# rampasek/GraphGPS

Hardware: NVIDIA H100
Metric: graphs/sec GPSLayer fwd+bwd (higher is better)
Workload: dtype f32

## Files before the change

### graphgps_b200/csrc/attention.cu

```cuda
#include "kernels.cuh"

namespace gps {

namespace {

constexpr int kWarpsPerBlock = 4;

__device__ __forceinline__ int find_graph(const int* __restrict__ gptr, int B, int node) {
  int lo = 0, hi = B;
  while (hi - lo > 1) {
    int mid = (lo + hi) >> 1;
    if (gptr[mid] <= node) lo = mid; else hi = mid;
  }
  return lo;
}

template <int LPR>
__device__ __forceinline__ float group_sum(float v) {
#pragma unroll
  for (int o = LPR / 2; o > 0; o >>= 1) v += __shfl_xor_sync(0xffffffffu, v, o);
  return v;
}

__device__ __forceinline__ int warp_max_i(int v) {
#pragma unroll
  for (int o = 16; o > 0; o >>= 1) v = max(v, __shfl_xor_sync(0xffffffffu, v, o));
  return v;
}

struct DropQuad {
  Philox4 r;
  uint32_t thr;
  float keep_scale;
};
__device__ __forceinline__ void drop_quad_refresh(DropQuad& q, float p, uint64_t seed, uint64_t offset, int head, int i, int jl) {
  q.r = philox4x32(seed, offset + (uint64_t)(GPS_SITE_ATTN_P + head), ((uint64_t)i << 20) | (uint64_t)(jl >> 2));
}
__device__ __forceinline__ float drop_quad_scale(const DropQuad& q, int jl) {
  const int k = jl & 3;
  const uint32_t bits = k == 0 ? q.r.v[0] : k == 1 ? q.r.v[1] : k == 2 ? q.r.v[2] : q.r.v[3];
  return bits >= q.thr ? q.keep_scale : 0.f;
}
__device__ __forceinline__ void drop_quad_init(DropQuad& q, float p) {
  q.thr = (uint32_t)fminf(p * 4294967296.f, 4294967295.f);
  q.keep_scale = 1.f / (1.f - p);
}

template <int VW> struct VecT;
template <> struct VecT<4> { using T = float4; };
template <> struct VecT<1> { using T = float; };

template <int VW> __device__ __forceinline__ typename VecT<VW>::T vld(const float* p);
template <> __device__ __forceinline__ float4 vld<4>(const float* p) { return ld4(p); }
template <> __device__ __forceinline__ float vld<1>(const float* p) { return *p; }
template <int VW> __device__ __forceinline__ typename VecT<VW>::T vzero();
template <> __device__ __forceinline__ float4 vzero<4>() { return f4zero(); }
template <> __device__ __forceinline__ float vzero<1>() { return 0.f; }
__device__ __forceinline__ void vst(float* p, float4 v) { st4(p, v); }
__device__ __forceinline__ void vst(float* p, float v) { *p = v; }
__device__ __forceinline__ float4 vscale(float4 a, float s) { return f4scale(a, s); }
__device__ __forceinline__ float vscale(float a, float s) { return a * s; }
__device__ __forceinline__ float vdot(float4 a, float4 b) { return a.x * b.x + a.y * b.y + a.z * b.z + a.w * b.w; }
__device__ __forceinline__ float vdot(float a, float b) { return a * b; }
__device__ __forceinline__ void vplanes_store(const Planes& p, int64_t r, int64_t c, float4 v) { planes_store4(p, r, c, v); }
__device__ __forceinline__ void vplanes_store(const Planes& p, int64_t r, int64_t c, float v) {
  const __nv_bfloat16 h = __float2bfloat16_rn(v);
  p.hi[r * p.ld + c] = h;
  if (p.lo) p.lo[r * p.ld + c] = __float2bfloat16_rn(v - __bfloat162float(h));
}

template <int CH, int LPR, int VW>
__device__ __forceinline__ void load_slice(typename VecT<VW>::T* dst, const float* row, int sub, int nch, bool ok) {
#pragma unroll
  for (int c = 0; c < CH; ++c) {
    int ch = sub + c * LPR;
    dst[c] = (ok && ch < nch) ? vld<VW>(row + ch * VW) : vzero<VW>();
  }
}
template <int CH, int LPR, int VW>
__device__ __forceinline__ void store_slice(const typename VecT<VW>::T* src, float* row, int sub, int nch) {
#pragma unroll
  for (int c = 0; c < CH; ++c) {
    int ch = sub + c * LPR;
    if (ch < nch) vst(row + ch * VW, src[c]);
  }
}
template <int CH, int LPR, int VW>
__device__ __forceinline__ void store_slice_planes(const typename VecT<VW>::T* src, const Planes& p, int64_t r, int64_t col0,
                                                   int sub, int nch) {
  if (!p.hi) return;
#pragma unroll
  for (int c = 0; c < CH; ++c) {
    int ch = sub + c * LPR;
    if (ch < nch) vplanes_store(p, r, col0 + ch * VW, src[c]);
  }
}
template <int CH, typename V>
__device__ __forceinline__ float dot_slice(const V* a, const V* b) {
  float s = 0.f;
#pragma unroll
  for (int c = 0; c < CH; ++c) s += vdot(a[c], b[c]);
  return s;
}

struct AttnArgs {
  const int* gptr; int B; int N; int H; int hd;
  const float* Q; const float* K; const float* V; int64_t ld;
  float* O; const float* Oc; const float* dO; int64_t ldo;
  float* lse; const float* lsec; float* delta; const float* deltac;
  float* dQ; float* dK; float* dV; int64_t ldg;
  float scale; float p_drop; uint64_t seed, offset;
  const unsigned long long* offset_dev;
  Planes Op, dQp, dKp, dVp;
  int smem_rows;
  const float* bias; int64_t nmax; float* gbias;
};
__device__ __forceinline__ uint64_t eff_offset(const AttnArgs& a) {
  return a.offset + ((a.p_drop > 0.f && a.offset_dev) ? *a.offset_dev : 0ull);
}

struct StagedRows {
  const float* x; int64_t ldx;
  const float* y; int64_t ldy;
};
template <int RPB, int VW>
__device__ __forceinline__ StagedRows stage_rows(const AttnArgs& a, const float* X, int64_t ldX, const float* Y, int64_t ldY,
                                                 int h, float* sm) {
  const int64_t hoff = (int64_t)h * a.hd;
  StagedRows r{X + hoff, ldX, Y + hoff, ldY};
  const int r0 = blockIdx.x * RPB;
  if (a.smem_rows <= 0 || r0 >= a.N) return r;
  const int last = min(r0 + RPB, a.N) - 1;
  const int kmin = a.gptr[find_graph(a.gptr, a.B, r0)];
  const int R = a.gptr[find_graph(a.gptr, a.B, last) + 1] - kmin;
  if (R > a.smem_rows) return r;
  const int pitch = a.hd + 4, nch = VW == 4 ? a.hd >> 2 : a.hd;
  float* sx = sm;
  float* sy = sm + (int64_t)a.smem_rows * pitch;
  for (int idx = threadIdx.x; idx < R * nch; idx += blockDim.x) {
    const int row = idx / nch, c = idx - row * nch;
    vst(sx + row * pitch + c * VW, vld<VW>(X + (int64_t)(kmin + row) * ldX + hoff + c * VW));
    vst(sy + row * pitch + c * VW, vld<VW>(Y + (int64_t)(kmin + row) * ldY + hoff + c * VW));
  }
  __syncthreads();
  r.x = sx - (int64_t)kmin * pitch; r.ldx = pitch;
  r.y = sy - (int64_t)kmin * pitch; r.ldy = pitch;
  return r;
}

template <int CH, int LPR, bool BIAS, int VW>
__global__ void __launch_bounds__(kWarpsPerBlock * 32) k_attn_fwd(AttnArgs a) {
  extern __shared__ float attn_sm[];
  using V = typename VecT<VW>::T;
  constexpr int RPW = 32 / LPR;
  const int warp = threadIdx.x >> 5, lane = threadIdx.x & 31;
  const int sub = lane % LPR, rloc = lane / LPR;
  const int h = blockIdx.y;
  const int i = (blockIdx.x * kWarpsPerBlock + warp) * RPW + rloc;
  const bool row_ok = i < a.N;
  const int nch = a.hd / VW;
  const uint64_t offs = eff_offset(a);
  int gs = 0, n = 0;
  const float* brow = nullptr;
  if (row_ok) {
    int g = find_graph(a.gptr, a.B, i);
    gs = a.gptr[g];
    n = a.gptr[g + 1] - gs;
    if constexpr (BIAS) brow = a.bias + (((int64_t)g * a.H + h) * a.nmax + (i - gs)) * a.nmax;
  }
  const int nloop = warp_max_i(n);
  const int64_t hoff = (int64_t)h * a.hd;
  V q[CH], o[CH];
  load_slice<CH, LPR, VW>(q, a.Q + (int64_t)(row_ok ? i : 0) * a.ld + hoff, sub, nch, row_ok);
#pragma unroll
  for (int c = 0; c < CH; ++c) {
    q[c] = vscale(q[c], a.scale);
    o[c] = vzero<VW>();
  }
  float m = -INFINITY, l = 0.f;
  const bool use_drop = a.p_drop > 0.f;
  DropQuad dq;
  drop_quad_init(dq, a.p_drop);
  const StagedRows kv = stage_rows<RPW * kWarpsPerBlock, VW>(a, a.K, a.ld, a.V, a.ld, h, attn_sm);
  V kc[CH], vc[CH];
  load_slice<CH, LPR, VW>(kc, kv.x + (int64_t)gs * kv.ldx, sub, nch, n > 0);
  load_slice<CH, LPR, VW>(vc, kv.y + (int64_t)gs * kv.ldy, sub, nch, n > 0);
  float bc = 0.f;
  if constexpr (BIAS) bc = n > 0 ? brow[0] : 0.f;
  for (int jl = 0; jl < nloop; ++jl) {
    if (use_drop && (jl & 3) == 0) drop_quad_refresh(dq, a.p_drop, a.seed, offs, h, i, jl);
    const bool valid = jl < n;
    const bool nvalid = jl + 1 < n;
    const int jn = gs + (nvalid ? jl + 1 : 0);
    V kn[CH], vn[CH];
    load_slice<CH, LPR, VW>(kn, kv.x + (int64_t)jn * kv.ldx, sub, nch, nvalid);
    load_slice<CH, LPR, VW>(vn, kv.y + (int64_t)jn * kv.ldy, sub, nch, nvalid);
    float bn = 0.f;
    if constexpr (BIAS) bn = nvalid ? brow[jl + 1] : 0.f;
    float s = group_sum<LPR>(dot_slice<CH>(q, kc));
    if constexpr (BIAS) s += bc;
    s = valid ? s : -INFINITY;
    const float m_new = fmaxf(m, s);
    const float corr = (m_new == -INFINITY) ? 1.f : __expf(m - m_new);
    const float p = valid ? __expf(s - m_new) : 0.f;
    l = l * corr + p;
    const float pd = use_drop ? p * drop_quad_scale(dq, jl) : p;
#pragma unroll
    for (int c = 0; c < CH; ++c) {
      if constexpr (VW == 4) {
        o[c].x = o[c].x * corr + pd * vc[c].x;
        o[c].y = o[c].y * corr + pd * vc[c].y;
        o[c].z = o[c].z * corr + pd * vc[c].z;
        o[c].w = o[c].w * corr + pd * vc[c].w;
      } else {
        o[c] = o[c] * corr + pd * vc[c];
      }
      kc[c] = kn[c];
      vc[c] = vn[c];
    }
    if constexpr (BIAS) bc = bn;
    m = m_new;
  }
  if (row_ok) {
    const float inv = 1.f / l;
#pragma unroll
    for (int c = 0; c < CH; ++c) o[c] = vscale(o[c], inv);
    store_slice<CH, LPR, VW>(o, a.O + (int64_t)i * a.ldo + hoff, sub, nch);
    store_slice_planes<CH, LPR, VW>(o, a.Op, i, hoff, sub, nch);
    if (sub == 0) a.lse[(int64_t)i * a.H + h] = m + __logf(l);
  }
}

template <int VW>
__global__ void k_attn_delta(AttnArgs a) {
  using V = typename VecT<VW>::T;
  const int64_t t = ((int64_t)blockIdx.x * blockDim.x + threadIdx.x) >> 3;
  const int sub = threadIdx.x & 7;
  const bool ok = t < (int64_t)a.N * a.H;
  const int64_t i = ok ? t / a.H : 0;
  const int h = ok ? (int)(t - i * a.H) : 0;
  const V* go = reinterpret_cast<const V*>(a.dO + i * a.ldo + (int64_t)h * a.hd);
  const V* oo = reinterpret_cast<const V*>(a.Oc + i * a.ldo + (int64_t)h * a.hd);
  float acc = 0.f;
  if (ok)
    for (int c = sub; c < a.hd / VW; c += 8) {
      const V x = __ldg(go + c), y = __ldg(oo + c);
      acc += vdot(x, y);
    }
  acc += __shfl_xor_sync(0xffffffffu, acc, 4);
  acc += __shfl_xor_sync(0xffffffffu, acc, 2);
  acc += __shfl_xor_sync(0xffffffffu, acc, 1);
  if (ok && sub == 0) a.delta[t] = acc;
}

template <int CH, int LPR, bool BIAS, int VW>
__device__ __forceinline__ void attn_bwd_q_body(const AttnArgs& a, float* attn_sm) {
  using V = typename VecT<VW>::T;
  constexpr int RPW = 32 / LPR;
  const int warp = threadIdx.x >> 5, lane = threadIdx.x & 31;
  const int sub = lane % LPR, rloc = lane / LPR;
  const int h = blockIdx.y;
  const int i = (blockIdx.x * kWarpsPerBlock + warp) * RPW + rloc;
  const bool row_ok = i < a.N;
  const int nch = a.hd / VW;
  const uint64_t offs = eff_offset(a);
  int gs = 0, n = 0;
  int64_t brow = 0;
  if (row_ok) {
    int g = find_graph(a.gptr, a.B, i);
    gs = a.gptr[g];
    n = a.gptr[g + 1] - gs;
    if constexpr (BIAS) brow = (((int64_t)g * a.H + h) * a.nmax + (i - gs)) * a.nmax;
  }
  const int nloop = warp_max_i(n);
  const int64_t hoff = (int64_t)h * a.hd;
  const int ir = row_ok ? i : 0;
  V q[CH], go[CH], gq[CH];
  load_slice<CH, LPR, VW>(q, a.Q + (int64_t)ir * a.ld + hoff, sub, nch, row_ok);
  load_slice<CH, LPR, VW>(go, a.dO + (int64_t)ir * a.ldo + hoff, sub, nch, row_ok);
  {
    const float dl = row_ok ? a.deltac[(int64_t)i * a.H + h] : 0.f;
#pragma unroll
    for (int c = 0; c < CH; ++c) gq[c] = vzero<VW>();
    const float lse = row_ok ? a.lsec[(int64_t)i * a.H + h] : 0.f;
#pragma unroll
    for (int c = 0; c < CH; ++c) q[c] = vscale(q[c], a.scale);
    const bool use_drop = a.p_drop > 0.f;
    DropQuad dq;
    drop_quad_init(dq, a.p_drop);
    const StagedRows kv = stage_rows<RPW * kWarpsPerBlock, VW>(a, a.K, a.ld, a.V, a.ld, h, attn_sm);
    V kk[CH], vv[CH];
    load_slice<CH, LPR, VW>(kk, kv.x + (int64_t)gs * kv.ldx, sub, nch, n > 0);
    load_slice<CH, LPR, VW>(vv, kv.y + (int64_t)gs * kv.ldy, sub, nch, n > 0);
    float bc = 0.f;
    if constexpr (BIAS) bc = n > 0 ? a.bias[brow] : 0.f;
    for (int jl = 0; jl < nloop; ++jl) {
      if (use_drop && (jl & 3) == 0) drop_quad_refresh(dq, a.p_drop, a.seed, offs, h, i, jl);
      const bool valid = jl < n;
      const bool nvalid = jl + 1 < n;
      const int jn = gs + (nvalid ? jl + 1 : 0);
      V kn[CH], vn[CH];
      load_slice<CH, LPR, VW>(kn, kv.x + (int64_t)jn * kv.ldx, sub, nch, nvalid);
      load_slice<CH, LPR, VW>(vn, kv.y + (int64_t)jn * kv.ldy, sub, nch, nvalid);
      float bn = 0.f;
      if constexpr (BIAS) bn = nvalid ? a.bias[brow + jl + 1] : 0.f;
      float s = dot_slice<CH>(q, kk), dp = dot_slice<CH>(go, vv);
#pragma unroll
      for (int ofs = LPR / 2; ofs > 0; ofs >>= 1) {
        s += __shfl_xor_sync(0xffffffffu, s, ofs);
        dp += __shfl_xor_sync(0xffffffffu, dp, ofs);
      }
      if constexpr (BIAS) s += bc;
      const float p = valid ? __expf(s - lse) : 0.f;
      const float ds = p * (dp * (use_drop ? drop_quad_scale(dq, jl) : 1.f) - dl);
      if constexpr (BIAS) {
        if (a.gbias && valid && sub == 0) a.gbias[brow + jl] = ds;
        bc = bn;
      }
#pragma unroll
      for (int c = 0; c < CH; ++c) {
        if constexpr (VW == 4) {
          gq[c].x += ds * kk[c].x;
          gq[c].y += ds * kk[c].y;
          gq[c].z += ds * kk[c].z;
          gq[c].w += ds * kk[c].w;
        } else {
          gq[c] += ds * kk[c];
        }
        kk[c] = kn[c];
        vv[c] = vn[c];
      }
    }
  }
  if (row_ok) {
#pragma unroll
    for (int c = 0; c < CH; ++c) gq[c] = vscale(gq[c], a.scale);
    store_slice<CH, LPR, VW>(gq, a.dQ + (int64_t)i * a.ldg + hoff, sub, nch);
    store_slice_planes<CH, LPR, VW>(gq, a.dQp, i, hoff, sub, nch);
  }
}

template <int CH, int LPR, bool BIAS, int VW>
__device__ __forceinline__ void attn_bwd_kv_body(const AttnArgs& a, float* attn_sm) {
  using V = typename VecT<VW>::T;
  constexpr int RPW = 32 / LPR;
  const int warp = threadIdx.x >> 5, lane = threadIdx.x & 31;
  const int sub = lane % LPR, rloc = lane / LPR;
  const int h = blockIdx.y;
  const int j = (blockIdx.x * kWarpsPerBlock + warp) * RPW + rloc;
  const bool row_ok = j < a.N;
  const int nch = a.hd / VW;
  const uint64_t offs = eff_offset(a);
  int gs = 0, n = 0;
  const float* bcol = nullptr;
  if (row_ok) {
    int g = find_graph(a.gptr, a.B, j);
    gs = a.gptr[g];
    n = a.gptr[g + 1] - gs;
    if constexpr (BIAS) bcol = a.bias + ((int64_t)g * a.H + h) * a.nmax * a.nmax + (j - gs);
  }
  const int nloop = warp_max_i(n);
  const int jl = j - gs;
  const int64_t hoff = (int64_t)h * a.hd;
  const int jr = row_ok ? j : 0;
  V kk[CH], vv[CH], gk[CH], gv[CH];
  load_slice<CH, LPR, VW>(kk, a.K + (int64_t)jr * a.ld + hoff, sub, nch, row_ok);
  load_slice<CH, LPR, VW>(vv, a.V + (int64_t)jr * a.ld + hoff, sub, nch, row_ok);
#pragma unroll
  for (int c = 0; c < CH; ++c) {
    gk[c] = vzero<VW>();
    gv[c] = vzero<VW>();
  }
  const StagedRows qd = stage_rows<RPW * kWarpsPerBlock, VW>(a, a.Q, a.ld, a.dO, a.ldo, h, attn_sm);
  V q[CH], go[CH];
  load_slice<CH, LPR, VW>(q, qd.x + (int64_t)gs * qd.ldx, sub, nch, n > 0);
  load_slice<CH, LPR, VW>(go, qd.y + (int64_t)gs * qd.ldy, sub, nch, n > 0);
  for (int il = 0; il < nloop; ++il) {
    const bool valid = il < n;
    const int i = gs + (valid ? il : 0);
    const bool nvalid = il + 1 < n;
    const int in_ = gs + (nvalid ? il + 1 : 0);
    V qn[CH], gon[CH];
    load_slice<CH, LPR, VW>(qn, qd.x + (int64_t)in_ * qd.ldx, sub, nch, nvalid);
    load_slice<CH, LPR, VW>(gon, qd.y + (int64_t)in_ * qd.ldy, sub, nch, nvalid);
    float s = dot_slice<CH>(q, kk), dp = dot_slice<CH>(go, vv);
#pragma unroll
    for (int ofs = LPR / 2; ofs > 0; ofs >>= 1) {
      s += __shfl_xor_sync(0xffffffffu, s, ofs);
      dp += __shfl_xor_sync(0xffffffffu, dp, ofs);
    }
    const float lse = valid ? a.lsec[(int64_t)i * a.H + h] : 0.f;
    const float dl = valid ? a.deltac[(int64_t)i * a.H + h] : 0.f;
    float p;
    if constexpr (BIAS) p = valid ? __expf(s * a.scale + bcol[(int64_t)il * a.nmax] - lse) : 0.f;
    else p = valid ? __expf(s * a.scale - lse) : 0.f;
    float dsc = 1.f;
    if (a.p_drop > 0.f) {
      DropQuad dq;
      drop_quad_init(dq, a.p_drop);
      drop_quad_refresh(dq, a.p_drop, a.seed, offs, h, i, jl);
      dsc = drop_quad_scale(dq, jl);
    }
    const float pd = p * dsc;
    const float ds = p * (dp * dsc - dl) * a.scale;
#pragma unroll
    for (int c = 0; c < CH; ++c) {
      if constexpr (VW == 4) {
        gk[c].x += ds * q[c].x; gk[c].y += ds * q[c].y; gk[c].z += ds * q[c].z; gk[c].w += ds * q[c].w;
        gv[c].x += pd * go[c].x; gv[c].y += pd * go[c].y; gv[c].z += pd * go[c].z; gv[c].w += pd * go[c].w;
      } else {
        gk[c] += ds * q[c];
        gv[c] += pd * go[c];
      }
      q[c] = qn[c];
      go[c] = gon[c];
    }
  }
  if (row_ok) {
    store_slice<CH, LPR, VW>(gk, a.dK + (int64_t)j * a.ldg + hoff, sub, nch);
    store_slice<CH, LPR, VW>(gv, a.dV + (int64_t)j * a.ldg + hoff, sub, nch);
    store_slice_planes<CH, LPR, VW>(gk, a.dKp, j, hoff, sub, nch);
    store_slice_planes<CH, LPR, VW>(gv, a.dVp, j, hoff, sub, nch);
  }
}

template <int CH, int LPR, bool BIAS, int VW>
__global__ void __launch_bounds__(kWarpsPerBlock * 32) k_attn_bwd(AttnArgs a) {
  extern __shared__ float attn_sm[];
  if (blockIdx.z == 0) attn_bwd_kv_body<CH, LPR, BIAS, VW>(a, attn_sm);
  else attn_bwd_q_body<CH, LPR, BIAS, VW>(a, attn_sm);
}

enum { KFWD = 0, KBWD = 1 };

constexpr int kStageBytes = 72 * 1024;

static bool attn_vec4(const AttnArgs& a, int which) {
  return a.hd % 4 == 0 && a.ld % 4 == 0 && a.ldo % 4 == 0 && (which == KFWD || a.ldg % 4 == 0);
}

template <int CH, int LPR, bool BIAS, int VW>
static void launch_one(int which, const AttnArgs& a0, cudaStream_t stream) {
  constexpr int RPW = 32 / LPR;
  AttnArgs a = a0;
  static const bool stage_on = [] {
    const char* e = getenv("GPS_B200_ATTN_STAGE");
    return e && e[0] == '1';
  }();
  const int pitch = a.hd + 4;
  a.smem_rows = (stage_on && a.B > 0 && a.N < 64LL * a.B) ? kStageBytes / (2 * pitch * 4) : 0;
  const size_t smem = a.smem_rows > 0 ? (size_t)2 * a.smem_rows * pitch * 4 : 0;
  static bool attr_done[2] = {false, false};
  if (smem > 0 && !attr_done[which]) {
    if (which == KFWD)
      cudaFuncSetAttribute(k_attn_fwd<CH, LPR, BIAS, VW>, cudaFuncAttributeMaxDynamicSharedMemorySize, kStageBytes);
    else cudaFuncSetAttribute(k_attn_bwd<CH, LPR, BIAS, VW>, cudaFuncAttributeMaxDynamicSharedMemorySize, kStageBytes);
    attr_done[which] = true;
  }
  dim3 grid((unsigned)ceil_div(a.N, (int64_t)RPW * kWarpsPerBlock), (unsigned)a.H, which == KFWD ? 1 : 2);
  dim3 block(kWarpsPerBlock * 32);
  if (which == KFWD) k_attn_fwd<CH, LPR, BIAS, VW><<<grid, block, smem, stream>>>(a);
  else k_attn_bwd<CH, LPR, BIAS, VW><<<grid, block, smem, stream>>>(a);
}

static int dispatch(int which, const AttnArgs& a, cudaStream_t stream) {
  GPS_REQUIRE(a.hd > 0 && a.hd <= 192, GPS_ERR_UNSUPPORTED, "attention: head dim %d must be in 1..192", a.hd);
  if (a.N == 0) return GPS_OK;
  const int vw = attn_vec4(a, which) ? 4 : 1;
  const int nch = a.hd / vw;
  int lpr = 1;
  while ((nch + lpr - 1) / lpr > 6) lpr *= 2;
  const int ch = (nch + lpr - 1) / lpr;
#define GPS_ATTN_CASE(VWV, CHV, LPRV)                                  \
  if (vw == VWV && ch == CHV && lpr == LPRV) {                         \
    if (a.bias) launch_one<CHV, LPRV, true, VWV>(which, a, stream);    \
    else launch_one<CHV, LPRV, false, VWV>(which, a, stream);          \
    GPS_LAUNCH_CHECK();                                                \
    return GPS_OK;                                                     \
  }
  GPS_ATTN_CASE(4, 1, 1) GPS_ATTN_CASE(4, 2, 1) GPS_ATTN_CASE(4, 3, 1) GPS_ATTN_CASE(4, 4, 1) GPS_ATTN_CASE(4, 5, 1)
  GPS_ATTN_CASE(4, 6, 1) GPS_ATTN_CASE(4, 4, 2) GPS_ATTN_CASE(4, 5, 2) GPS_ATTN_CASE(4, 6, 2) GPS_ATTN_CASE(4, 4, 4)
  GPS_ATTN_CASE(4, 5, 4) GPS_ATTN_CASE(4, 6, 4) GPS_ATTN_CASE(4, 4, 8) GPS_ATTN_CASE(4, 5, 8) GPS_ATTN_CASE(4, 6, 8)
  GPS_ATTN_CASE(1, 1, 1) GPS_ATTN_CASE(1, 2, 1) GPS_ATTN_CASE(1, 3, 1) GPS_ATTN_CASE(1, 4, 1) GPS_ATTN_CASE(1, 5, 1)
  GPS_ATTN_CASE(1, 6, 1) GPS_ATTN_CASE(1, 4, 2) GPS_ATTN_CASE(1, 5, 2) GPS_ATTN_CASE(1, 6, 2) GPS_ATTN_CASE(1, 4, 4)
  GPS_ATTN_CASE(1, 5, 4) GPS_ATTN_CASE(1, 6, 4) GPS_ATTN_CASE(1, 4, 8) GPS_ATTN_CASE(1, 5, 8) GPS_ATTN_CASE(1, 6, 8)
  GPS_ATTN_CASE(1, 4, 16) GPS_ATTN_CASE(1, 5, 16) GPS_ATTN_CASE(1, 6, 16) GPS_ATTN_CASE(1, 4, 32)
  GPS_ATTN_CASE(1, 5, 32) GPS_ATTN_CASE(1, 6, 32)
#undef GPS_ATTN_CASE
  set_error("attention: no kernel for head dim %d", a.hd);
  return GPS_ERR_UNSUPPORTED;
}

}

int attention_fwd(const GpsGraph& g, int64_t heads, int64_t hd, const float* Q, const float* K, const float* V,
                  int64_t ld, float* O, int64_t ldo, float* lse, float p_drop, uint64_t seed, uint64_t offset,
                  cudaStream_t stream, const unsigned long long* offset_dev, Planes Op, const GpsAttnBias* bias) {
  AttnArgs a{};
  a.offset_dev = offset_dev;
  a.Op = Op;
  if (bias) { a.bias = bias->bias; a.nmax = bias->nmax; }
  a.gptr = g.graph_ptr; a.B = (int)g.B; a.N = (int)g.N; a.H = (int)heads; a.hd = (int)hd;
  a.Q = Q; a.K = K; a.V = V; a.ld = ld; a.O = O; a.ldo = ldo; a.lse = lse;
  a.scale = 1.f / sqrtf((float)hd); a.p_drop = p_drop; a.seed = seed; a.offset = offset;
  return dispatch(KFWD, a, stream);
}

int attention_bwd(const GpsGraph& g, int64_t heads, int64_t hd, const float* Q, const float* K, const float* V,
                  int64_t ld, const float* O, const float* dO, int64_t ldo, const float* lse, float* delta,
                  float* dQ, float* dK, float* dV, int64_t ldg, float p_drop, uint64_t seed, uint64_t offset,
                  cudaStream_t stream, const unsigned long long* offset_dev, Planes dQp, Planes dKp, Planes dVp,
                  const GpsAttnBias* bias) {
  AttnArgs a{};
  a.offset_dev = offset_dev;
  if (bias) { a.bias = bias->bias; a.nmax = bias->nmax; a.gbias = bias->grad_bias; }
  a.dQp = dQp; a.dKp = dKp; a.dVp = dVp;
  a.gptr = g.graph_ptr; a.B = (int)g.B; a.N = (int)g.N; a.H = (int)heads; a.hd = (int)hd;
  a.Q = Q; a.K = K; a.V = V; a.ld = ld; a.Oc = O; a.dO = dO; a.ldo = ldo; a.lsec = lse;
  a.delta = delta; a.deltac = delta; a.dQ = dQ; a.dK = dK; a.dV = dV; a.ldg = ldg;
  a.scale = 1.f / sqrtf((float)hd); a.p_drop = p_drop; a.seed = seed; a.offset = offset;
  if (a.gbias)
    GPS_CUDA(cudaMemsetAsync(a.gbias, 0, (size_t)(g.B * heads * a.nmax * a.nmax) * sizeof(float), stream));
  GPS_REQUIRE(a.hd > 0 && a.hd <= 192, GPS_ERR_UNSUPPORTED, "attention: head dim %d must be in 1..192", a.hd);
  if (a.N == 0) return GPS_OK;
  const int64_t nt = (int64_t)a.N * a.H * 8;
  if (attn_vec4(a, KBWD)) k_attn_delta<4><<<(unsigned)ceil_div(nt, (int64_t)256), 256, 0, stream>>>(a);
  else k_attn_delta<1><<<(unsigned)ceil_div(nt, (int64_t)256), 256, 0, stream>>>(a);
  GPS_LAUNCH_CHECK();
  return dispatch(KBWD, a, stream);
}

}
```

Before: 340,100.

## Add graph-owned block attention kernels staging K/V in shared memory for small graphs

Replaces the env-gated per-block K/V staging with new kernels where each block owns whole graphs, found by a cooperative search over the graph pointers, and stages their K/V (or Q/dO) in shared memory. The backward merges the dQ and dK/dV passes into one kernel, caching per-pair ds and p values in shared memory so the dK/dV pass reads them instead of recomputing the softmax. This path is on by default when mean graph size is below 32 nodes, and falls back to the direct global-memory row kernels when a window's graphs do not fit. It adds extra syncs, a fixed shared-memory footprint that may lower occupancy, and a serial fallback path when capacity is exceeded.

Result: faster. 349,900 (median of 6 runs) (+2.9%).

```diff
diff --git a/graphgps_b200/csrc/attention.cu b/graphgps_b200/csrc/attention.cu
--- a/graphgps_b200/csrc/attention.cu
+++ b/graphgps_b200/csrc/attention.cu
@@ -112,52 +112,16 @@
   float scale; float p_drop; uint64_t seed, offset;
   const unsigned long long* offset_dev;
   Planes Op, dQp, dKp, dVp;
-  int smem_rows;
   const float* bias; int64_t nmax; float* gbias;
 };
 __device__ __forceinline__ uint64_t eff_offset(const AttnArgs& a) {
   return a.offset + ((a.p_drop > 0.f && a.offset_dev) ? *a.offset_dev : 0ull);
 }
 
-struct StagedRows {
-  const float* x; int64_t ldx;
-  const float* y; int64_t ldy;
-};
-template <int RPB, int VW>
-__device__ __forceinline__ StagedRows stage_rows(const AttnArgs& a, const float* X, int64_t ldX, const float* Y, int64_t ldY,
-                                                 int h, float* sm) {
-  const int64_t hoff = (int64_t)h * a.hd;
-  StagedRows r{X + hoff, ldX, Y + hoff, ldY};
-  const int r0 = blockIdx.x * RPB;
-  if (a.smem_rows <= 0 || r0 >= a.N) return r;
-  const int last = min(r0 + RPB, a.N) - 1;
-  const int kmin = a.gptr[find_graph(a.gptr, a.B, r0)];
-  const int R = a.gptr[find_graph(a.gptr, a.B, last) + 1] - kmin;
-  if (R > a.smem_rows) return r;
-  const int pitch = a.hd + 4, nch = VW == 4 ? a.hd >> 2 : a.hd;
-  float* sx = sm;
-  float* sy = sm + (int64_t)a.smem_rows * pitch;
-  for (int idx = threadIdx.x; idx < R * nch; idx += blockDim.x) {
-    const int row = idx / nch, c = idx - row * nch;
-    vst(sx + row * pitch + c * VW, vld<VW>(X + (int64_t)(kmin + row) * ldX + hoff + c * VW));
-    vst(sy + row * pitch + c * VW, vld<VW>(Y + (int64_t)(kmin + row) * ldY + hoff + c * VW));
-  }
-  __syncthreads();
-  r.x = sx - (int64_t)kmin * pitch; r.ldx = pitch;
-  r.y = sy - (int64_t)kmin * pitch; r.ldy = pitch;
-  return r;
-}
-
-template <int CH, int LPR, bool BIAS, int VW>
-__global__ void __launch_bounds__(kWarpsPerBlock * 32) k_attn_fwd(AttnArgs a) {
-  extern __shared__ float attn_sm[];
+template <int CH, int LPR, bool BIAS, int VW, bool PIPE>
+__device__ __forceinline__ void attn_fwd_row(const AttnArgs& a, int h, int i, bool row_ok) {
   using V = typename VecT<VW>::T;
-  constexpr int RPW = 32 / LPR;
-  const int warp = threadIdx.x >> 5, lane = threadIdx.x & 31;
-  const int sub = lane % LPR, rloc = lane / LPR;
-  const int h = blockIdx.y;
-  const int i = (blockIdx.x * kWarpsPerBlock + warp) * RPW + rloc;
-  const bool row_ok = i < a.N;
+  const int sub = (threadIdx.x & 31) % LPR;
   const int nch = a.hd / VW;
   const uint64_t offs = eff_offset(a);
   int gs = 0, n = 0;
@@ -181,10 +145,9 @@
   const bool use_drop = a.p_drop > 0.f;
   DropQuad dq;
   drop_quad_init(dq, a.p_drop);
-  const StagedRows kv = stage_rows<RPW * kWarpsPerBlock, VW>(a, a.K, a.ld, a.V, a.ld, h, attn_sm);
   V kc[CH], vc[CH];
-  load_slice<CH, LPR, VW>(kc, kv.x + (int64_t)gs * kv.ldx, sub, nch, n > 0);
-  load_slice<CH, LPR, VW>(vc, kv.y + (int64_t)gs * kv.ldy, sub, nch, n > 0);
+  load_slice<CH, LPR, VW>(kc, a.K + (int64_t)gs * a.ld + hoff, sub, nch, n > 0);
+  load_slice<CH, LPR, VW>(vc, a.V + (int64_t)gs * a.ld + hoff, sub, nch, n > 0);
   float bc = 0.f;
   if constexpr (BIAS) bc = n > 0 ? brow[0] : 0.f;
   for (int jl = 0; jl < nloop; ++jl) {
@@ -193,8 +156,13 @@
     const bool nvalid = jl + 1 < n;
     const int jn = gs + (nvalid ? jl + 1 : 0);
     V kn[CH], vn[CH];
-    load_slice<CH, LPR, VW>(kn, kv.x + (int64_t)jn * kv.ldx, sub, nch, nvalid);
-    load_slice<CH, LPR, VW>(vn, kv.y + (int64_t)jn * kv.ldy, sub, nch, nvalid);
+    if constexpr (PIPE) {
+      load_slice<CH, LPR, VW>(kn, a.K + (int64_t)jn * a.ld + hoff, sub, nch, nvalid);
+      load_slice<CH, LPR, VW>(vn, a.V + (int64_t)jn * a.ld + hoff, sub, nch, nvalid);
+    } else {
+      load_slice<CH, LPR, VW>(kc, a.K + (int64_t)(gs + (valid ? jl : 0)) * a.ld + hoff, sub, nch, valid);
+      load_slice<CH, LPR, VW>(vc, a.V + (int64_t)(gs + (valid ? jl : 0)) * a.ld + hoff, sub, nch, valid);
+    }
     float bn = 0.f;
     if constexpr (BIAS) bn = nvalid ? brow[jl + 1] : 0.f;
     float s = group_sum<LPR>(dot_slice<CH>(q, kc));
@@ -215,8 +183,10 @@
       } else {
         o[c] = o[c] * corr + pd * vc[c];
       }
-      kc[c] = kn[c];
-      vc[c] = vn[c];
+      if constexpr (PIPE) {
+        kc[c] = kn[c];
+        vc[c] = vn[c];
+      }
     }
     if constexpr (BIAS) bc = bn;
     m = m_new;
@@ -253,15 +223,10 @@
   if (ok && sub == 0) a.delta[t] = acc;
 }
 
-template <int CH, int LPR, bool BIAS, int VW>
-__device__ __forceinline__ void attn_bwd_q_body(const AttnArgs& a, float* attn_sm) {
+template <int CH, int LPR, bool BIAS, int VW, bool PIPE>
+__device__ __forceinline__ void attn_bwd_q_row(const AttnArgs& a, int h, int i, bool row_ok) {
   using V = typename VecT<VW>::T;
-  constexpr int RPW = 32 / LPR;
-  const int warp = threadIdx.x >> 5, lane = threadIdx.x & 31;
-  const int sub = lane % LPR, rloc = lane / LPR;
-  const int h = blockIdx.y;
-  const int i = (blockIdx.x * kWarpsPerBlock + warp) * RPW + rloc;
-  const bool row_ok = i < a.N;
+  const int sub = (threadIdx.x & 31) % LPR;
   const int nch = a.hd / VW;
   const uint64_t offs = eff_offset(a);
   int gs = 0, n = 0;
@@ -288,10 +253,9 @@
     const bool use_drop = a.p_drop > 0.f;
     DropQuad dq;
     drop_quad_init(dq, a.p_drop);
-    const StagedRows kv = stage_rows<RPW * kWarpsPerBlock, VW>(a, a.K, a.ld, a.V, a.ld, h, attn_sm);
     V kk[CH], vv[CH];
-    load_slice<CH, LPR, VW>(kk, kv.x + (int64_t)gs * kv.ldx, sub, nch, n > 0);
-    load_slice<CH, LPR, VW>(vv, kv.y + (int64_t)gs * kv.ldy, sub, nch, n > 0);
+    load_slice<CH, LPR, VW>(kk, a.K + (int64_t)gs * a.ld + hoff, sub, nch, n > 0);
+    load_slice<CH, LPR, VW>(vv, a.V + (int64_t)gs * a.ld + hoff, sub, nch, n > 0);
     float bc = 0.f;
     if constexpr (BIAS) bc = n > 0 ? a.bias[brow] : 0.f;
     for (int jl = 0; jl < nloop; ++jl) {
@@ -300,8 +264,13 @@
       const bool nvalid = jl + 1 < n;
       const int jn = gs + (nvalid ? jl + 1 : 0);
       V kn[CH], vn[CH];
-      load_slice<CH, LPR, VW>(kn, kv.x + (int64_t)jn * kv.ldx, sub, nch, nvalid);
-      load_slice<CH, LPR, VW>(vn, kv.y + (int64_t)jn * kv.ldy, sub, nch, nvalid);
+      if constexpr (PIPE) {
+        load_slice<CH, LPR, VW>(kn, a.K + (int64_t)jn * a.ld + hoff, sub, nch, nvalid);
+        load_slice<CH, LPR, VW>(vn, a.V + (int64_t)jn * a.ld + hoff, sub, nch, nvalid);
+      } else {
+        load_slice<CH, LPR, VW>(kk, a.K + (int64_t)(gs + (valid ? jl : 0)) * a.ld + hoff, sub, nch, valid);
+        load_slice<CH, LPR, VW>(vv, a.V + (int64_t)(gs + (valid ? jl : 0)) * a.ld + hoff, sub, nch, valid);
+      }
       float bn = 0.f;
       if constexpr (BIAS) bn = nvalid ? a.bias[brow + jl + 1] : 0.f;
       float s = dot_slice<CH>(q, kk), dp = dot_slice<CH>(go, vv);
@@ -327,8 +296,10 @@
         } else {
           gq[c] += ds * kk[c];
         }
-        kk[c] = kn[c];
-        vv[c] = vn[c];
+        if constexpr (PIPE) {
+          kk[c] = kn[c];
+          vv[c] = vn[c];
+        }
       }
     }
   }
@@ -340,15 +311,10 @@
   }
 }
 
-template <int CH, int LPR, bool BIAS, int VW>
-__device__ __forceinline__ void attn_bwd_kv_body(const AttnArgs& a, float* attn_sm) {
+template <int CH, int LPR, bool BIAS, int VW, bool PIPE>
+__device__ __forceinline__ void attn_bwd_kv_row(const AttnArgs& a, int h, int j, bool row_ok) {
   using V = typename VecT<VW>::T;
-  constexpr int RPW = 32 / LPR;
-  const int warp = threadIdx.x >> 5, lane = threadIdx.x & 31;
-  const int sub = lane % LPR, rloc = lane / LPR;
-  const int h = blockIdx.y;
-  const int j = (blockIdx.x * kWarpsPerBlock + warp) * RPW + rloc;
-  const bool row_ok = j < a.N;
+  const int sub = (threadIdx.x & 31) % LPR;
   const int nch = a.hd / VW;
   const uint64_t offs = eff_offset(a);
   int gs = 0, n = 0;
@@ -371,18 +337,22 @@
     gk[c] = vzero<VW>();
     gv[c] = vzero<VW>();
   }
-  const StagedRows qd = stage_rows<RPW * kWarpsPerBlock, VW>(a, a.Q, a.ld, a.dO, a.ldo, h, attn_sm);
   V q[CH], go[CH];
-  load_slice<CH, LPR, VW>(q, qd.x + (int64_t)gs * qd.ldx, sub, nch, n > 0);
-  load_slice<CH, LPR, VW>(go, qd.y + (int64_t)gs * qd.ldy, sub, nch, n > 0);
+  load_slice<CH, LPR, VW>(q, a.Q + (int64_t)gs * a.ld + hoff, sub, nch, n > 0);
+  load_slice<CH, LPR, VW>(go, a.dO + (int64_t)gs * a.ldo + hoff, sub, nch, n > 0);
   for (int il = 0; il < nloop; ++il) {
     const bool valid = il < n;
     const int i = gs + (valid ? il : 0);
     const bool nvalid = il + 1 < n;
     const int in_ = gs + (nvalid ? il + 1 : 0);
     V qn[CH], gon[CH];
-    load_slice<CH, LPR, VW>(qn, qd.x + (int64_t)in_ * qd.ldx, sub, nch, nvalid);
-    load_slice<CH, LPR, VW>(gon, qd.y + (int64_t)in_ * qd.ldy, sub, nch, nvalid);
+    if constexpr (PIPE) {
+      load_slice<CH, LPR, VW>(qn, a.Q + (int64_t)in_ * a.ld + hoff, sub, nch, nvalid);
+      load_slice<CH, LPR, VW>(gon, a.dO + (int64_t)in_ * a.ldo + hoff, sub, nch, nvalid);
+    } else {
+      load_slice<CH, LPR, VW>(q, a.Q + (int64_t)i * a.ld + hoff, sub, nch, valid);
+      load_slice<CH, LPR, VW>(go, a.dO + (int64_t)i * a.ldo + hoff, sub, nch, valid);
+    }
     float s = dot_slice<CH>(q, kk), dp = dot_slice<CH>(go, vv);
 #pragma unroll
     for (int ofs = LPR / 2; ofs > 0; ofs >>= 1) {
@@ -412,8 +382,10 @@
         gk[c] += ds * q[c];
         gv[c] += pd * go[c];
       }
-      q[c] = qn[c];
-      go[c] = gon[c];
+      if constexpr (PIPE) {
+        q[c] = qn[c];
+        go[c] = gon[c];
+      }
     }
   }
   if (row_ok) {
@@ -425,42 +397,350 @@
 }
 
 template <int CH, int LPR, bool BIAS, int VW>
+__global__ void __launch_bounds__(kWarpsPerBlock * 32) k_attn_fwd(AttnArgs a) {
+  const int i = (blockIdx.x * kWarpsPerBlock + (threadIdx.x >> 5)) * (32 / LPR) + (threadIdx.x & 31) / LPR;
+  attn_fwd_row<CH, LPR, BIAS, VW, true>(a, blockIdx.y, i, i < a.N);
+}
+
+template <int CH, int LPR, bool BIAS, int VW>
 __global__ void __launch_bounds__(kWarpsPerBlock * 32) k_attn_bwd(AttnArgs a) {
-  extern __shared__ float attn_sm[];
-  if (blockIdx.z == 0) attn_bwd_kv_body<CH, LPR, BIAS, VW>(a, attn_sm);
-  else attn_bwd_q_body<CH, LPR, BIAS, VW>(a, attn_sm);
+  const int i = (blockIdx.x * kWarpsPerBlock + (threadIdx.x >> 5)) * (32 / LPR) + (threadIdx.x & 31) / LPR;
+  if (blockIdx.z == 0) attn_bwd_kv_row<CH, LPR, BIAS, VW, true>(a, blockIdx.y, i, i < a.N);
+  else attn_bwd_q_row<CH, LPR, BIAS, VW, true>(a, blockIdx.y, i, i < a.N);
+}
+
+constexpr int kOwnRows = 64;
+constexpr int kStageFloats = 2 * 64 * 80;
+constexpr int kPairCap = 2048;
+
+__host__ __device__ inline int own_pitch(int hd, int vw) { return vw == 4 ? hd + 4 : hd + 1; }
+__host__ __device__ inline int own_cap(int pitch) {
+  return kStageFloats / (2 * pitch) < kOwnRows ? kStageFloats / (2 * pitch) : kOwnRows;
+}
+static size_t own_smem_bytes(int cap, int pitch, int pair_bufs) {
+  return ((size_t)2 * cap * pitch + (size_t)pair_bufs * kPairCap) * sizeof(float) + (size_t)4 * cap * sizeof(int);
+}
+
+__device__ __forceinline__ int2 first_graphs_at(const int* __restrict__ gptr, int B, int x0, int x1) {
+  int lo0 = 0, hi0 = B, lo1 = 0, hi1 = B;
+  while (hi0 > lo0 || hi1 > lo1) {
+    const int st0 = (hi0 - lo0 + blockDim.x - 1) / blockDim.x, st1 = (hi1 - lo1 + blockDim.x - 1) / blockDim.x;
+    const int c0 = lo0 + threadIdx.x * st0, c1 = lo1 + threadIdx.x * st1;
+    const int n0 = __syncthreads_count(c0 < hi0 && gptr[c0] < x0);
+    const int n1 = __syncthreads_count(c1 < hi1 && gptr[c1] < x1);
+    if (hi0 > lo0) { hi0 = min(hi0, lo0 + n0 * st0); lo0 = n0 > 0 ? lo0 + (n0 - 1) * st0 + 1 : lo0; }
+    if (hi1 > lo1) { hi1 = min(hi1, lo1 + n1 * st1); lo1 = n1 > 0 ? lo1 + (n1 - 1) * st1 + 1 : lo1; }
+  }
+  return make_int2(lo0, lo1);
+}
+
+struct OwnRows {
+  int r0, nr;
+  bool staged;
+};
+template <bool PAIRS>
+__device__ __forceinline__ OwnRows own_rows(const AttnArgs& a, int cap, int win, int* s_g, int* s_gs, int* s_n, int* s_po) {
+  __shared__ int s_total;
+  const int2 gg = first_graphs_at(a.gptr, a.B, blockIdx.x * win, (blockIdx.x + 1) * win);
+  const int g0 = gg.x, g1 = gg.y;
+  const int r0 = a.gptr[g0], nr = a.gptr[g1] - r0;
+  if (nr == 0 || nr > cap) return {r0, nr, false};
+  for (int g = g0 + threadIdx.x; g < g1; g += blockDim.x) {
+    const int gs = a.gptr[g], ge = a.gptr[g + 1];
+    for (int r = gs; r < ge; ++r) {
+      s_g[r - r0] = g;
+      s_gs[r - r0] = gs - r0;
+      s_n[r - r0] = ge - gs;
+    }
+  }
+  __syncthreads();
+  if constexpr (!PAIRS) return {r0, nr, true};
+  if (threadIdx.x < 32) {
+    const int lane = threadIdx.x, l0 = 2 * lane, l1 = l0 + 1;
+    const int c0 = l0 < nr ? s_n[l0] : 0, c1 = l1 < nr ? s_n[l1] : 0;
+    int v = c0 + c1;
+#pragma unroll
+    for (int o = 1; o < 32; o <<= 1) {
+      const int u = __shfl_up_sync(0xffffffffu, v, o);
+      if (lane >= o) v += u;
+    }
+    if (l0 < nr) s_po[l0] = v - c0 - c1;
+    if (l1 < nr) s_po[l1] = v - c1;
+    if (lane == 31) s_total = v;
+  }
+  __syncthreads();
+  return {r0, nr, s_total <= kPairCap};
+}
+
+template <int VW>
+__device__ __forceinline__ void own_stage(float* sx, float* sy, int pitch, const float* X, int64_t ldx, const float* Y,
+                                          int64_t ldy, int r0, int nr, int nch) {
+  for (int idx = threadIdx.x; idx < nr * nch; idx += blockDim.x) {
+    const int row = idx / nch, c = idx - row * nch;
+    vst(sx + row * pitch + c * VW, vld<VW>(X + (int64_t)(r0 + row) * ldx + c * VW));
+    vst(sy + row * pitch + c * VW, vld<VW>(Y + (int64_t)(r0 + row) * ldy + c * VW));
+  }
+  __syncthreads();
+}
+
+template <int CH, int LPR, bool BIAS, int VW>
+__global__ void __launch_bounds__(kWarpsPerBlock * 32) k_attn_fwd_own(AttnArgs a, int cap, int win, int pitch) {
+  extern __shared__ float4 own_sm[];
+  using V = typename VecT<VW>::T;
+  constexpr int RPW = 32 / LPR, RPB = RPW * kWarpsPerBlock;
+  const int warp = threadIdx.x >> 5, lane = threadIdx.x & 31;
+  const int sub = lane % LPR, rloc = lane / LPR;
+  const int h = blockIdx.y;
+  float* sk = reinterpret_cast<float*>(own_sm);
+  float* sv = sk + cap * pitch;
+  int* s_g = reinterpret_cast<int*>(sv + cap * pitch);
+  int *s_gs = s_g + cap, *s_n = s_g + 2 * cap;
+  const OwnRows own = own_rows<false>(a, cap, win, s_g, s_gs, s_n, nullptr);
+  if (!own.staged) {
+    for (int base = own.r0; base < own.r0 + own.nr; base += RPB) {
+      const int i = base + warp * RPW + rloc;
+      attn_fwd_row<CH, LPR, BIAS, VW, false>(a, h, i, i < own.r0 + own.nr);
+    }
+    return;
+  }
+  const int nch = a.hd / VW;
+  const int64_t hoff = (int64_t)h * a.hd;
+  own_stage<VW>(sk, sv, pitch, a.K + hoff, a.ld, a.V + hoff, a.ld, own.r0, own.nr, nch);
+  const uint64_t offs = eff_offset(a);
+  const bool use_drop = a.p_drop > 0.f;
+  DropQuad dq;
+  drop_quad_init(dq, a.p_drop);
+  for (int base = 0; base < own.nr; base += RPB) {
+    const int l = base + warp * RPW + rloc;
+    const bool row_ok = l < own.nr;
+    const int i = own.r0 + l;
+    const int n = row_ok ? s_n[l] : 0, gsl = row_ok ? s_gs[l] : 0;
+    const int nloop = warp_max_i(n);
+    const float* brow = nullptr;
+    if constexpr (BIAS)
+      if (row_ok) brow = a.bias + (((int64_t)s_g[l] * a.H + h) * a.nmax + (l - gsl)) * a.nmax;
+    V q[CH], o[CH];
+    load_slice<CH, LPR, VW>(q, a.Q + (int64_t)(row_ok ? i : own.r0) * a.ld + hoff, sub, nch, row_ok);
+#pragma unroll
+    for (int c = 0; c < CH; ++c) {
+      q[c] = vscale(q[c], a.scale);
+      o[c] = vzero<VW>();
+    }
+    float m = -INFINITY, l_sum = 0.f;
+    for (int jl = 0; jl < nloop; ++jl) {
+      if (use_drop && (jl & 3) == 0) drop_quad_refresh(dq, a.p_drop, a.seed, offs, h, i, jl);
+      const bool valid = jl < n;
+      const int jr = gsl + (valid ? jl : 0);
+      V kc[CH], vc[CH];
+      load_slice<CH, LPR, VW>(kc, sk + jr * pitch, sub, nch, true);
+      load_slice<CH, LPR, VW>(vc, sv + jr * pitch, sub, nch, true);
+      float s = group_sum<LPR>(dot_slice<CH>(q, kc));
+      if constexpr (BIAS) s += valid ? brow[jl] : 0.f;
+      s = valid ? s : -INFINITY;
+      const float m_new = fmaxf(m, s);
+      const float corr = (m_new == -INFINITY) ? 1.f : __expf(m - m_new);
+      const float p = valid ? __expf(s - m_new) : 0.f;
+      l_sum = l_sum * corr + p;
+      const float pd = use_drop ? p * drop_quad_scale(dq, jl) : p;
+#pragma unroll
+      for (int c = 0; c < CH; ++c) {
+        if constexpr (VW == 4) {
+          o[c].x = o[c].x * corr + pd * vc[c].x;
+          o[c].y = o[c].y * corr + pd * vc[c].y;
+          o[c].z = o[c].z * corr + pd * vc[c].z;
+          o[c].w = o[c].w * corr + pd * vc[c].w;
+        } else {
+          o[c] = o[c] * corr + pd * vc[c];
+        }
+      }
+      m = m_new;
+    }
+    if (row_ok) {
+      const float inv = 1.f / l_sum;
+#pragma unroll
+      for (int c = 0; c < CH; ++c) o[c] = vscale(o[c], inv);
+      store_slice<CH, LPR, VW>(o, a.O + (int64_t)i * a.ldo + hoff, sub, nch);
+      store_slice_planes<CH, LPR, VW>(o, a.Op, i, hoff, sub, nch);
+      if (sub == 0) a.lse[(int64_t)i * a.H + h] = m + __logf(l_sum);
+    }
+  }
+}
+
+template <int CH, int LPR, bool BIAS, int VW>
+__global__ void __launch_bounds__(kWarpsPerBlock * 32) k_attn_bwd_own(AttnArgs a, int cap, int win, int pitch) {
+  extern __shared__ float4 own_sm[];
+  using V = typename VecT<VW>::T;
+  constexpr int RPW = 32 / LPR, RPB = RPW * kWarpsPerBlock;
+  const int warp = threadIdx.x >> 5, lane = threadIdx.x & 31;
+  const int sub = lane % LPR, rloc = lane / LPR;
+  const int h = blockIdx.y;
+  float* sx = reinterpret_cast<float*>(own_sm);
+  float* sy = sx + cap * pitch;
+  float* sds = sy + cap * pitch;
+  float* spm = sds + kPairCap;
+  int* s_g = reinterpret_cast<int*>(spm + kPairCap);
+  int *s_gs = s_g + cap, *s_n = s_g + 2 * cap, *s_po = s_g + 3 * cap;
+  const OwnRows own = own_rows<true>(a, cap, win, s_g, s_gs, s_n, s_po);
+  if (!own.staged) {
+    for (int base = own.r0; base < own.r0 + own.nr; base += RPB) {
+      const int i = base + warp * RPW + rloc;
+      attn_bwd_q_row<CH, LPR, BIAS, VW, false>(a, h, i, i < own.r0 + own.nr);
+    }
+    for (int base = own.r0; base < own.r0 + own.nr; base += RPB) {
+      const int j = base + warp * RPW + rloc;
+      attn_bwd_kv_row<CH, LPR, BIAS, VW, false>(a, h, j, j < own.r0 + own.nr);
+    }
+    return;
+  }
+  const int nch = a.hd / VW;
+  const int64_t hoff = (int64_t)h * a.hd;
+  own_stage<VW>(sx, sy, pitch, a.K + hoff, a.ld, a.V + hoff, a.ld, own.r0, own.nr, nch);
+  const uint64_t offs = eff_offset(a);
+  const bool use_drop = a.p_drop > 0.f;
+  DropQuad dq;
+  drop_quad_init(dq, a.p_drop);
+  for (int base = 0; base < own.nr; base += RPB) {
+    const int l = base + warp * RPW + rloc;
+    const bool row_ok = l < own.nr;
+    const int i = own.r0 + l, ir = row_ok ? i : own.r0;
+    const int n = row_ok ? s_n[l] : 0, gsl = row_ok ? s_gs[l] : 0, po = row_ok ? s_po[l] : 0;
+    const int nloop = warp_max_i(n);
+    int64_t brow = 0;
+    if constexpr (BIAS)
+      if (row_ok) brow = (((int64_t)s_g[l] * a.H + h) * a.nmax + (l - gsl)) * a.nmax;
+    V qr[CH], q[CH], go[CH], gq[CH];
+    load_slice<CH, LPR, VW>(qr, a.Q + (int64_t)ir * a.ld + hoff, sub, nch, row_ok);
+    load_slice<CH, LPR, VW>(go, a.dO + (int64_t)ir * a.ldo + hoff, sub, nch, row_ok);
+#pragma unroll
+    for (int c = 0; c < CH; ++c) {
+      q[c] = vscale(qr[c], a.scale);
+      gq[c] = vzero<VW>();
+    }
+    const float dl = row_ok ? a.deltac[(int64_t)i * a.H + h] : 0.f;
+    const float lse = row_ok ? a.lsec[(int64_t)i * a.H + h] : 0.f;
+    for (int jl = 0; jl < nloop; ++jl) {
+      if (use_drop && (jl & 3) == 0) drop_quad_refresh(dq, a.p_drop, a.seed, offs, h, i, jl);
+      const bool valid = jl < n;
+      const int jr = gsl + (valid ? jl : 0);
+      V kk[CH], vv[CH];
+      load_slice<CH, LPR, VW>(kk, sx + jr * pitch, sub, nch, true);
+      load_slice<CH, LPR, VW>(vv, sy + jr * pitch, sub, nch, true);
+      float s = dot_slice<CH>(q, kk), dp = dot_slice<CH>(go, vv), sr = dot_slice<CH>(qr, kk);
+#pragma unroll
+      for (int ofs = LPR / 2; ofs > 0; ofs >>= 1) {
+        s += __shfl_xor_sync(0xffffffffu, s, ofs);
+        dp += __shfl_xor_sync(0xffffffffu, dp, ofs);
+        sr += __shfl_xor_sync(0xffffffffu, sr, ofs);
+      }
+      float bij = 0.f;
+      if constexpr (BIAS) bij = valid ? a.bias[brow + jl] : 0.f;
+      if constexpr (BIAS) s += bij;
+      const float p = valid ? __expf(s - lse) : 0.f;
+      const float dsc = use_drop ? drop_quad_scale(dq, jl) : 1.f;
+      const float ds = p * (dp * dsc - dl);
+      if (valid && sub == 0) {
+        float pk;
+        if constexpr (BIAS) pk = __expf(sr * a.scale + bij - lse);
+        else pk = __expf(sr * a.scale - lse);
+        sds[po + jl] = pk * (dp * dsc - dl) * a.scale;
+        spm[po + jl] = pk * dsc;
+        if constexpr (BIAS)
+          if (a.gbias) a.gbias[brow + jl] = ds;
+      }
+#pragma unroll
+      for (int c = 0; c < CH; ++c) {
+        if constexpr (VW == 4) {
+          gq[c].x += ds * kk[c].x;
+          gq[c].y += ds * kk[c].y;
+          gq[c].z += ds * kk[c].z;
+          gq[c].w += ds * kk[c].w;
+        } else {
+          gq[c] += ds * kk[c];
+        }
+      }
+    }
+    if (row_ok) {
+#pragma unroll
+      for (int c = 0; c < CH; ++c) gq[c] = vscale(gq[c], a.scale);
+      store_slice<CH, LPR, VW>(gq, a.dQ + (int64_t)i * a.ldg + hoff, sub, nch);
+      store_slice_planes<CH, LPR, VW>(gq, a.dQp, i, hoff, sub, nch);
+    }
+  }
+  __syncthreads();
+  own_stage<VW>(sx, sy, pitch, a.Q + hoff, a.ld, a.dO + hoff, a.ldo, own.r0, own.nr, nch);
+  for (int base = 0; base < own.nr; base += RPB) {
+    const int l = base + warp * RPW + rloc;
+    const bool row_ok = l < own.nr;
+    const int j = own.r0 + l;
+    const int n = row_ok ? s_n[l] : 0, gsl = row_ok ? s_gs[l] : 0;
+    const int jl = l - gsl;
+    const int pcol = row_ok ? s_po[l] - jl * n + jl : 0;
+    const int nloop = warp_max_i(n);
+    V gk[CH], gv[CH];
+#pragma unroll
+    for (int c = 0; c < CH; ++c) {
+      gk[c] = vzero<VW>();
+      gv[c] = vzero<VW>();
+    }
+    for (int il = 0; il < nloop; ++il) {
+      const bool valid = il < n;
+      const int ir = gsl + (valid ? il : 0);
+      const float ds = valid ? sds[pcol + il * n] : 0.f;
+      const float pd = valid ? spm[pcol + il * n] : 0.f;
+      V q[CH], go[CH];
+      load_slice<CH, LPR, VW>(q, sx + ir * pitch, sub, nch, true);
+      load_slice<CH, LPR, VW>(go, sy + ir * pitch, sub, nch, true);
+#pragma unroll
+      for (int c = 0; c < CH; ++c) {
+        if constexpr (VW == 4) {
+          gk[c].x += ds * q[c].x; gk[c].y += ds * q[c].y; gk[c].z += ds * q[c].z; gk[c].w += ds * q[c].w;
+          gv[c].x += pd * go[c].x; gv[c].y += pd * go[c].y; gv[c].z += pd * go[c].z; gv[c].w += pd * go[c].w;
+        } else {
+          gk[c] += ds * q[c];
+          gv[c] += pd * go[c];
+        }
+      }
+    }
+    if (row_ok) {
+      store_slice<CH, LPR, VW>(gk, a.dK + (int64_t)j * a.ldg + hoff, sub, nch);
+      store_slice<CH, LPR, VW>(gv, a.dV + (int64_t)j * a.ldg + hoff, sub, nch);
+      store_slice_planes<CH, LPR, VW>(gk, a.dKp, j, hoff, sub, nch);
+      store_slice_planes<CH, LPR, VW>(gv, a.dVp, j, hoff, sub, nch);
+    }
+  }
 }
 
 enum { KFWD = 0, KBWD = 1 };
 
-constexpr int kStageBytes = 72 * 1024;
+constexpr int kOwnMeanMax = 32;
 
 static bool attn_vec4(const AttnArgs& a, int which) {
   return a.hd % 4 == 0 && a.ld % 4 == 0 && a.ldo % 4 == 0 && (which == KFWD || a.ldg % 4 == 0);
 }
 
 template <int CH, int LPR, bool BIAS, int VW>
-static void launch_one(int which, const AttnArgs& a0, cudaStream_t stream) {
+static void launch_one(int which, const AttnArgs& a, cudaStream_t stream) {
   constexpr int RPW = 32 / LPR;
-  AttnArgs a = a0;
-  static const bool stage_on = [] {
-    const char* e = getenv("GPS_B200_ATTN_STAGE");
-    return e && e[0] == '1';
-  }();
-  const int pitch = a.hd + 4;
-  a.smem_rows = (stage_on && a.B > 0 && a.N < 64LL * a.B) ? kStageBytes / (2 * pitch * 4) : 0;
-  const size_t smem = a.smem_rows > 0 ? (size_t)2 * a.smem_rows * pitch * 4 : 0;
-  static bool attr_done[2] = {false, false};
-  if (smem > 0 && !attr_done[which]) {
-    if (which == KFWD)
-      cudaFuncSetAttribute(k_attn_fwd<CH, LPR, BIAS, VW>, cudaFuncAttributeMaxDynamicSharedMemorySize, kStageBytes);
-    else cudaFuncSetAttribute(k_attn_bwd<CH, LPR, BIAS, VW>, cudaFuncAttributeMaxDynamicSharedMemorySize, kStageBytes);
-    attr_done[which] = true;
-  }
-  dim3 grid((unsigned)ceil_div(a.N, (int64_t)RPW * kWarpsPerBlock), (unsigned)a.H, which == KFWD ? 1 : 2);
-  dim3 block(kWarpsPerBlock * 32);
-  if (which == KFWD) k_attn_fwd<CH, LPR, BIAS, VW><<<grid, block, smem, stream>>>(a);
-  else k_attn_bwd<CH, LPR, BIAS, VW><<<grid, block, smem, stream>>>(a);
+  const dim3 block(kWarpsPerBlock * 32);
+  if (a.B > 0 && a.N < (int64_t)kOwnMeanMax * a.B) {
+    const int pitch = own_pitch(a.hd, VW), cap = own_cap(pitch), win = cap / 2;
+    const size_t smem = own_smem_bytes(cap, pitch, which == KFWD ? 0 : 2);
+    static bool attr_done[2] = {false, false};
+    if (!attr_done[which]) {
+      const int bytes = (int)((kStageFloats + 2 * kPairCap) * sizeof(float) + 4 * kOwnRows * sizeof(int));
+      if (which == KFWD)
+        cudaFuncSetAttribute(k_attn_fwd_own<CH, LPR, BIAS, VW>, cudaFuncAttributeMaxDynamicSharedMemorySize, bytes);
+      else cudaFuncSetAttribute(k_attn_bwd_own<CH, LPR, BIAS, VW>, cudaFuncAttributeMaxDynamicSharedMemorySize, bytes);
+      attr_done[which] = true;
+    }
+    const dim3 grid((unsigned)ceil_div((int64_t)a.N, (int64_t)win), (unsigned)a.H);
+    if (which == KFWD) k_attn_fwd_own<CH, LPR, BIAS, VW><<<grid, block, smem, stream>>>(a, cap, win, pitch);
+    else k_attn_bwd_own<CH, LPR, BIAS, VW><<<grid, block, smem, stream>>>(a, cap, win, pitch);
+    return;
+  }
+  const dim3 grid((unsigned)ceil_div(a.N, (int64_t)RPW * kWarpsPerBlock), (unsigned)a.H, which == KFWD ? 1 : 2);
+  if (which == KFWD) k_attn_fwd<CH, LPR, BIAS, VW><<<grid, block, 0, stream>>>(a);
+  else k_attn_bwd<CH, LPR, BIAS, VW><<<grid, block, 0, stream>>>(a);
 }
 
 static int dispatch(int which, const AttnArgs& a, cudaStream_t stream) {
```
